# atsuki-ichikawa/KoeMorph

Measured on AMD Instinct MI355X. Metric: blendshape frames/sec (52-coef, 256-win, d_model=256), higher is better.
Workload: dtype f32; 1 GPU; C2: 256 windows/GPU x 136448 samples (8.5 s @16 kHz) -> 1024-pt STFT, hop 533, 80-bin log-mel (257 frames) -> dual-stream attention d_model=256, 8 heads, window 256 -> 52 coefficients + EMA; from audio resident in HBM (rotating batches); windows_per_gpu=256, samples_per_window=136448, parallelism=window-sharded x1, no collective

## Files before the change

koemorph_amd/csrc/km_api.hip:

```cpp
#include <hip/hip_runtime.h>

#include <cstdlib>

#include <cstring>
#include <vector>

#include "km_context.h"
#include "km_device.h"
#include "km_gemm.h"

using namespace km;

#define HIP_TRY(expr)                                                                         \
    do {                                                                                      \
        hipError_t e_ = (expr);                                                               \
        if (e_ != hipSuccess) {                                                                                                        \
            (void)hipGetLastError();  \
            return fail(KM_ERR_HIP, "%s: %s", #expr, hipGetErrorString(e_));                                                           \
        }                                                                                                                              \
    } while (0)

static int free_streams(Context* c);
static int free_train(Context* c);
static int free_pipeline(Context* c);
// ... 7 lines not shown
    return KM_OK;
}

static int need_dual(Context* c) {
    if (int rc = need_ready(c)) return rc;
    if (c->kind != 0) return fail(KM_ERR_INVALID_ARG, "this entry point needs a dual-stream handle (km_create), not a legacy one");
    return KM_OK;
}

static int need_legacy_train(Context* c, int64_t B) {
    if (int rc = need_ready(c)) return rc;
    if (c->kind != 1) return fail(KM_ERR_INVALID_ARG, "this entry point needs a legacy handle (km_legacy_create)");
    if (!c->tr_params || !c->ltr_ws) return fail(KM_ERR_NOT_FINALIZED, "call km_legacy_train_init first");
    if (B <= 0 || B > c->tr_windows) return fail(KM_ERR_WORKSPACE, "km_legacy_train_init sized the step for %lld windows, got %lld",
                                                 (long long)c->tr_windows, (long long)B);
    return KM_OK;
}

namespace km { LogParams plan_log_params(MelPlan* p); }

extern "C" {

int km_finalize(km_handle h, void* stream) {
    if (!h) return fail(KM_ERR_INVALID_ARG, "NULL handle");
    Context* c = h;
    int ndev = 0;
    if (hipGetDeviceCount(&ndev) != hipSuccess || ndev == 0)
        return fail(KM_ERR_HIP, "no HIP device: libkoemorph_hip has no CPU fallback");
    HIP_TRY(hipGetDevice(&c->device));
    if (!c->host_finalized)
        if (int rc = finalize_host(c)) return rc;
    for (auto& kv : c->packed) {
        Packed& p = kv.second;
        if (!p.dev) HIP_TRY(hipMalloc(reinterpret_cast<void**>(&p.dev), p.host.size() * sizeof(float)));
        HIP_TRY(hipMemcpyAsync(p.dev, p.host.data(), p.host.size() * sizeof(float), hipMemcpyHostToDevice,
                               (hipStream_t)stream));
    }
    HIP_TRY(hipStreamSynchronize((hipStream_t)stream));
    for (MelPlan* p : c->mel_plans)
        if (int rc = upload_mel_plan(p)) return rc;
    if (c->kind != 2)
        if (int rc = ensure_chunk_counters(c, 4096, stream)) return rc;
    c->dev_finalized = true;
    return KM_OK;
}

static int free_ws(Context* c) {
    if (c->ws_zemo) HIP_TRY(hipFree(c->ws_zemo));
    if (c->ws_zemo_win) HIP_TRY(hipFree(c->ws_zemo_win));
    if (c->ws_melpow) HIP_TRY(hipFree(c->ws_melpow));
    if (c->ws_melmax) HIP_TRY(hipFree(c->ws_melmax));
    if (c->ws_mel) HIP_TRY(hipFree(c->ws_mel));
    if (c->ws_short) HIP_TRY(hipFree(c->ws_short));
    if (c->ws_generic) HIP_TRY(hipFree(c->ws_generic));
    c->ws_zemo = c->ws_zemo_win = c->ws_melpow = c->ws_mel = c->ws_short = c->ws_generic = nullptr;
    c->ws_melmax = nullptr;
    c->ws_windows = c->ws_samples = c->ws_frames = 0;
    c->ws_mels = 0;
    return KM_OK;
}

int km_reserve(km_handle h, int64_t max_windows, int64_t max_samples) {
    if (!h || max_windows <= 0 || max_samples < 0) return fail(KM_ERR_INVALID_ARG, "km_reserve: bad argument");
    Context* c = h;
    if (c->kind == 2) return fail(KM_ERR_INVALID_ARG, "KoeMorphModel handles take no audio: use km_koemorph_reserve");
    int min_hop = c->cfg.mel.hop_length, max_mels = c->cfg.mel.n_mels;
// ... 1124 lines not shown
```

koemorph_amd/csrc/km_context.h:

```cpp
#pragma once

#include <cstdint>
#include <map>
#include <string>
#include <vector>

#include "koemorph.h"

namespace km {

constexpr int kNumMouth = 28;
constexpr int kNumExpr = 24;
extern const int kMouthIdx[kNumMouth];
extern const int kExprIdx[kNumExpr];

struct HostParam {
    std::vector<int64_t> shape;
    std::vector<float> data;
    bool loaded = false;
};

struct Packed {
    std::vector<float> host;
    float* dev = nullptr;
};

constexpr int kMelRpWaves = 8;
constexpr int kMelRpGroups = 4;
constexpr int kMelRpRow = 580;

struct MelPlan {
    km_mel_config cfg{};
    int n_freq = 0;
    std::vector<float> window;
    std::vector<float> twiddle;
    std::vector<int32_t> fb_start;
    std::vector<int32_t> fb_count;
    std::vector<int32_t> fb_offset;
    std::vector<float> fb_weight;
    std::vector<int32_t> fbg_gid;
    std::vector<int32_t> fbg_desc;
    std::vector<float> fbg_weight;
    int fbg_extent = 0;
    float* d_window = nullptr;
    float* d_twiddle = nullptr;
    int32_t* d_fb_start = nullptr;
    int32_t* d_fb_count = nullptr;
    int32_t* d_fb_offset = nullptr;
    float* d_fb_weight = nullptr;
    int32_t* d_fbg_gid = nullptr;
    int32_t* d_fbg_desc = nullptr;
    float* d_fbg_weight = nullptr;
    bool uploaded = false;
};

struct Options {
    int core_split = 0;
// ... 270 lines not shown
```

koemorph_amd/csrc/km_core.hip:

```cpp
#include <hip/hip_runtime.h>

#include <type_traits>

#include "km_context.h"
#include "km_device.h"

namespace km {

typedef float f32x4 __attribute__((ext_vector_type(4)));
#define KM_MFMA(a, b, c) __builtin_amdgcn_mfma_f32_16x16x4f32((a), (b), (c), 0, 0, 0)

#define HIP_TRY(expr)                                                                         \
    do {                                                                                      \
        hipError_t e_ = (expr);                                                               \
        if (e_ != hipSuccess) {                                                                                                        \
            (void)hipGetLastError();  \
            return fail(KM_ERR_HIP, "%s: %s", #expr, hipGetErrorString(e_));                                                           \
        }                                                                                                                              \
    } while (0)

namespace fused {
constexpr int D = 256, T = 256, NK = 80, NQ = 28, DH = 128;
constexpr int KT = 259, KTP = 264, YS = 264, NW = 8, NT = 512;
constexpr int KP = 33;
// ... 37 lines not shown
    const float* seq_edge;
    int seq_nfc, seq_stride, seq_n;
    const unsigned char* ready;
    unsigned char* started;
    const int* seq_start;
    int seq_min;
};

__device__ __forceinline__ int mouth_slot_of(int i) { return (i >= 14 && i <= 40) ? i - 14 : (i == 51 ? 27 : -1); }

template <bool ATTN, bool FUSE_DB, int NP = 0, bool TAB = false>
__global__ __launch_bounds__(512) void core_fused_kernel(CoreArgs a) {
    using namespace fused;
    extern __shared__ __attribute__((aligned(16))) float smem[];
    float* R1 = smem;
    float* R2 = smem + r1_floats(NP);

    const int b = blockIdx.x;
    const int tid = threadIdx.x;
    const int lane = tid & 63;
    const int wave = __builtin_amdgcn_readfirstlane(tid >> 6);
    const int g = lane >> 4, j = lane & 15;
    if constexpr (FUSE_DB) {
        if (a.ready && !a.ready[b]) return;
    }

    const int n0 = 32 * wave + j;
    float4 bw0 = make_float4(0.f, 0.f, 0.f, 0.f), bw1 = bw0;
    if constexpr (NP == 0) {
        const float4* wp0 = reinterpret_cast<const float4*>(a.wce_p) + (size_t)wave * KP * 64 + lane;
        bw0 = wp0[0];
    }
    const float bb0 = a.bce[n0], bb1 = a.bce[n0 + 16];
    const float g0 = a.ln_g[n0], g1 = a.ln_g[n0 + 16], be0 = a.ln_b[n0], be1 = a.ln_b[n0 + 16];
    float bf4[4], w24[4];
#pragma unroll
    for (int r = 0; r < 4; ++r) { bf4[r] = a.bf[16 * wave + 4 * g + r]; w24[r] = a.w2[16 * wave + 4 * g + r]; }
    const float tail_b2 = a.b2[0], tail_ws = tid < 52 ? a.wsum[tid] : 0.f;

    if constexpr (FUSE_DB) {
        float ref_db, floor_db;
        log_window_consts(a.lp, __uint_as_float(a.melmax[b]), ref_db, floor_db);
        const int F = a.n_frames;
        const int U = a.n_use;
        const int tv = U < T ? U : T;
        const float4* src = reinterpret_cast<const float4*>(a.melpow + (int64_t)b * F * NK);
        const float4 *seq_rows = nullptr, *seq_e = nullptr;
        if constexpr (TAB) {
            int r0 = a.seq_start[b];
            r0 = (r0 < 0 ? 0 : r0) - a.seq_min;
            r0 = r0 < 0 ? 0 : (r0 > a.seq_nfc - F ? a.seq_nfc - F : r0);
            seq_rows = reinterpret_cast<const float4*>(a.seq_pow + (int64_t)r0 * NK);
            seq_e = reinterpret_cast<const float4*>(a.seq_edge + (int64_t)b * 2 * NK);
        } else if (a.seq_pow) {
            const int64_t gw = a.win0 + b, clip = gw / a.seq_n, wi = gw - clip * a.seq_n;
            seq_rows = reinterpret_cast<const float4*>(a.seq_pow + (clip * a.seq_nfc + wi * a.seq_stride) * NK);
            seq_e = reinterpret_cast<const float4*>(a.seq_edge + gw * 2 * NK);
        }
        auto row4 = [&](int fr) -> const float4* {
            if (!seq_rows) return src + fr * 20;
            return fr == 0 ? seq_e : (fr == F - 1 ? seq_e + 20 : seq_rows + fr * 20);
        };
        float4* dst = reinterpret_cast<float4*>(R1);
        const float4 z4 = make_float4(0.f, 0.f, 0.f, 0.f);
        if constexpr (NP > 0) {
            auto src_row = [&](int t) -> int {
                if (t < T) return t < tv ? (t < F ? t : F - 1) : -1;
                if (t >= T + 3) return -1;
                const int r = t - T;
                int fr = -1;
                if (U >= 3) fr = U - 3 + r; else if (r < U) fr = r;
// ... 133 lines not shown
    } else {
        const float4* wp = reinterpret_cast<const float4*>(a.wce_p) + (size_t)wave * KP * 64 + lane;
        float4 bw = bw0;
        for (int kp = 0; kp < KP; ++kp) {
            const float4 bn = wp[(size_t)(kp + 1 < KP ? kp + 1 : kp) * 64];
#pragma unroll
            for (int ds = 0; ds < 2; ++ds) {
                const float* xr = R1 + (4 * (2 * kp + ds) + g) * NK + j;
                const float b0 = ds ? bw.z : bw.x, b1 = ds ? bw.w : bw.y;
                float av[5];
#pragma unroll
                for (int mt = 0; mt < 5; ++mt) av[mt] = xr[16 * mt];
#pragma unroll
                for (int mt = 0; mt < 5; ++mt) {
                    acc[mt][0] = KM_MFMA(av[mt], b0, acc[mt][0]);
                    acc[mt][1] = KM_MFMA(av[mt], b1, acc[mt][1]);
                }
            }
            bw = bn;
        }
    }
    f32x4 q0 = f32x4{0, 0, 0, 0}, q1 = q0, v0 = q0, v1 = q0;
    if constexpr (NP == 0) {
        const f32x4* qp0 = reinterpret_cast<const f32x4*>(a.qk_p) + (size_t)wave * KB * 2 * 64 + lane;
        const f32x4* vp0 = reinterpret_cast<const f32x4*>(a.wv_p) + (size_t)wave * KB * 2 * 64 + lane;
        q0 = qp0[0]; q1 = qp0[64]; v0 = vp0[0]; v1 = vp0[64];
    }
    {
#pragma unroll
        for (int mt = 0; mt < 5; ++mt)
#pragma unroll
            for (int r = 0; r < 4; ++r) { acc[mt][0][r] += bb0; acc[mt][1][r] += bb1; }
    }
    float mean[5][4], rstd[5][4];
#pragma unroll
    for (int pass = 0; pass < 2; ++pass) {
        float part[5][4];
#pragma unroll
        for (int mt = 0; mt < 5; ++mt)
#pragma unroll
            for (int r = 0; r < 4; ++r) {
                float v;
                if (pass == 0) {
                    v = acc[mt][0][r] + acc[mt][1][r];
                } else {
                    const float d0 = acc[mt][0][r] - mean[mt][r], d1 = acc[mt][1][r] - mean[mt][r];
                    v = d0 * d0 + d1 * d1;
                }
                part[mt][r] = row16_sum(v);
            }
        float* P = R2 + pass * (NW * NK);
        if (j == 0) {
#pragma unroll
            for (int mt = 0; mt < 5; ++mt)
#pragma unroll
                for (int r = 0; r < 4; ++r) P[(16 * mt + 4 * g + r) * NW + wave] = part[mt][r];
        }
        __syncthreads();
        float* Tt = R2 + 2 * NW * NK + pass * NK;
        if (lane < NK / NW) {
            const int row = wave * (NK / NW) + lane;
            const f32x4* pr = reinterpret_cast<const f32x4*>(P + row * NW);
            const f32x4 lo = pr[0], hi = pr[1];
            float s = 0.f;
            s += lo[0]; s += lo[1]; s += lo[2]; s += lo[3];
            s += hi[0]; s += hi[1]; s += hi[2]; s += hi[3];
            Tt[row] = s;
        }
        __syncthreads();
#pragma unroll
        for (int mt = 0; mt < 5; ++mt) {
            const f32x4 t4 = *reinterpret_cast<const f32x4*>(Tt + 16 * mt + 4 * g);
#pragma unroll
            for (int r = 0; r < 4; ++r) {
                if (pass == 0) mean[mt][r] = t4[r] * (1.0f / D);
                else rstd[mt][r] = __builtin_amdgcn_rsqf(t4[r] * (1.0f / D) + 1e-5f);
            }
        }
    }
    {
#pragma unroll
        for (int mt = 0; mt < 5; ++mt)
#pragma unroll
            for (int r = 0; r < 4; ++r) {
                const float y0 = (acc[mt][0][r] - mean[mt][r]) * rstd[mt][r] * g0 + be0;
                const float y1 = (acc[mt][1][r] - mean[mt][r]) * rstd[mt][r] * g1 + be1;
                if constexpr (NP == 0) {
                    float* yr = R1 + (16 * mt + 4 * g + r) * YS + n0;
                    yr[0] = y0;
                    yr[16] = y1;
                } else {
                    unsigned short* yp = reinterpret_cast<unsigned short*>(R1) + (16 * mt + 4 * g + r) * YSB + n0;
                    float r0 = y0, r1 = y1;
#pragma unroll
                    for (int pc = 0; pc < NP; ++pc) {
                        const __bf16 p0 = (__bf16)r0, p1 = (__bf16)r1;
                        yp[pc * (NK * YSB)] = __builtin_bit_cast(unsigned short, p0);
                        yp[pc * (NK * YSB) + 16] = __builtin_bit_cast(unsigned short, p1);
                        r0 -= (float)p0;
                        r1 -= (float)p1;
                    }
                }
            }
    }
    __syncthreads();

    f32x4 S[5][2], V[5][2];
#pragma unroll
    for (int mt = 0; mt < 5; ++mt) {
        S[mt][0] = f32x4{0, 0, 0, 0}; S[mt][1] = f32x4{0, 0, 0, 0};
        V[mt][0] = f32x4{0, 0, 0, 0}; V[mt][1] = f32x4{0, 0, 0, 0};
    }
    if constexpr (NP > 0) {
        const u32x4c* wp = reinterpret_cast<const u32x4c*>(a.qkv_s) + (size_t)wave * 8 * 4 * NP * 64 + lane;
        const unsigned short* Yp = reinterpret_cast<const unsigned short*>(R1) + j * YSB + 8 * g;
        u32x4c bw[4][NP];
#pragma unroll
        for (int t = 0; t < 4; ++t)
#pragma unroll
            for (int pc = 0; pc < NP; ++pc) bw[t][pc] = wp[(t * NP + pc) * 64];
        for (int kb = 0; kb < 8; ++kb) {
            const int kn = kb + 1 < 8 ? kb + 1 : kb;
            u32x4c bn[4][NP];
#pragma unroll
            for (int t = 0; t < 4; ++t)
#pragma unroll
                for (int pc = 0; pc < NP; ++pc) bn[t][pc] = wp[((kn * 4 + t) * NP + pc) * 64];
#pragma unroll
            for (int mt = 0; mt < 5; ++mt) {
                bf16x8 ap[NP];
#pragma unroll
                for (int pc = 0; pc < NP; ++pc)
                    ap[pc] = __builtin_bit_cast(bf16x8, *reinterpret_cast<const u32x4c*>(Yp + pc * (NK * YSB) + 16 * mt * YSB + 32 * kb));
#pragma unroll
                for (int t = 0; t < 4; ++t) {
                    f32x4 c4 = t < 2 ? S[mt][t] : V[mt][t - 2];
                    if constexpr (NP == 3) {
                        c4 = __builtin_amdgcn_mfma_f32_16x16x32_bf16(ap[1], __builtin_bit_cast(bf16x8, bw[t][1]), c4, 0, 0, 0);
                        c4 = __builtin_amdgcn_mfma_f32_16x16x32_bf16(ap[0], __builtin_bit_cast(bf16x8, bw[t][2]), c4, 0, 0, 0);
                        c4 = __builtin_amdgcn_mfma_f32_16x16x32_bf16(ap[2], __builtin_bit_cast(bf16x8, bw[t][0]), c4, 0, 0, 0);
                    }
                    c4 = __builtin_amdgcn_mfma_f32_16x16x32_bf16(ap[0], __builtin_bit_cast(bf16x8, bw[t][1]), c4, 0, 0, 0);
                    c4 = __builtin_amdgcn_mfma_f32_16x16x32_bf16(ap[1], __builtin_bit_cast(bf16x8, bw[t][0]), c4, 0, 0, 0);
                    c4 = __builtin_amdgcn_mfma_f32_16x16x32_bf16(ap[0], __builtin_bit_cast(bf16x8, bw[t][0]), c4, 0, 0, 0);
                    if (t < 2) S[mt][t] = c4; else V[mt][t - 2] = c4;
                }
            }
#pragma unroll
            for (int t = 0; t < 4; ++t)
#pragma unroll
                for (int pc = 0; pc < NP; ++pc) bw[t][pc] = bn[t][pc];
        }
    } else {
        const f32x4* qp = reinterpret_cast<const f32x4*>(a.qk_p) + (size_t)wave * KB * 2 * 64 + lane;
        const f32x4* vp = reinterpret_cast<const f32x4*>(a.wv_p) + (size_t)wave * KB * 2 * 64 + lane;
        for (int kb = 0; kb < KB; ++kb) {
            const int kn = kb + 1 < KB ? kb + 1 : kb;
            const f32x4 q0n = qp[(size_t)kn * 128], q1n = qp[(size_t)kn * 128 + 64];
            const f32x4 v0n = vp[(size_t)kn * 128], v1n = vp[(size_t)kn * 128 + 64];
            f32x4 ya[5];
#pragma unroll
            for (int mt = 0; mt < 5; ++mt)
                ya[mt] = *reinterpret_cast<const f32x4*>(R1 + (16 * mt + j) * YS + 16 * kb + 4 * g);
#pragma unroll
            for (int s = 0; s < 4; ++s)
#pragma unroll
                for (int mt = 0; mt < 5; ++mt) {
                    const float av = ya[mt][s];
                    S[mt][0] = KM_MFMA(av, q0[s], S[mt][0]);
                    S[mt][1] = KM_MFMA(av, q1[s], S[mt][1]);
                    V[mt][0] = KM_MFMA(av, v0[s], V[mt][0]);
                    V[mt][1] = KM_MFMA(av, v1[s], V[mt][1]);
                }
            q0 = q0n; q1 = q1n; v0 = v0n; v1 = v1n;
        }
    }
#pragma unroll
    for (int qt = 0; qt < 2; ++qt) {
        float m = S[0][qt][0];
#pragma unroll
        for (int mt = 0; mt < 5; ++mt)
#pragma unroll
            for (int r = 0; r < 4; ++r) m = fmaxf(m, S[mt][qt][r]);
        m = fmaxf(m, __shfl_xor(m, 16));
        m = fmaxf(m, __shfl_xor(m, 32));
        float sum = 0.f;
#pragma unroll
        for (int mt = 0; mt < 5; ++mt)
#pragma unroll
            for (int r = 0; r < 4; ++r) {
                const float e = __builtin_amdgcn_exp2f((S[mt][qt][r] - m) * 1.44269504088896341f);
                S[mt][qt][r] = e;
                sum += e;
            }
        sum += __shfl_xor(sum, 16);
        sum += __shfl_xor(sum, 32);
        const float inv = __builtin_amdgcn_rcpf(sum);
#pragma unroll
        for (int mt = 0; mt < 5; ++mt)
#pragma unroll
            for (int r = 0; r < 4; ++r) S[mt][qt][r] *= inv;
    }

    f32x4 O[2][2];
    O[0][0] = f32x4{0, 0, 0, 0}; O[0][1] = f32x4{0, 0, 0, 0};
    O[1][0] = f32x4{0, 0, 0, 0}; O[1][1] = f32x4{0, 0, 0, 0};
#pragma unroll
// ... 43 lines not shown
    Z[0] = f32x4{0, 0, 0, 0}; Z[1] = f32x4{0, 0, 0, 0};
    {
        const f32x4* fp = reinterpret_cast<const f32x4*>(a.wf_p) + (size_t)wave * KB * 64 + lane;
#pragma unroll 4
        for (int kb = 0; kb < KB; ++kb) {
            const f32x4 wa = fp[(size_t)kb * 64];
            const f32x4 o0 = *reinterpret_cast<const f32x4*>(R1 + j * YS + 16 * kb + 4 * g);
            const f32x4 o1 = *reinterpret_cast<const f32x4*>(R1 + (16 + j) * YS + 16 * kb + 4 * g);
#pragma unroll
            for (int s = 0; s < 4; ++s) {
                Z[0] = KM_MFMA(wa[s], o0[s], Z[0]);
                Z[1] = KM_MFMA(wa[s], o1[s], Z[1]);
            }
        }
    }
    {
        float zp[2] = {0.f, 0.f};
#pragma unroll
        for (int r = 0; r < 4; ++r) {
            const float bfv = bf4[r], w2v = w24[r];
            zp[0] += fmaxf(Z[0][r] + bfv, 0.f) * w2v;
            zp[1] += fmaxf(Z[1][r] + bfv, 0.f) * w2v;
        }
#pragma unroll
        for (int qt = 0; qt < 2; ++qt) {
            zp[qt] += __shfl_xor(zp[qt], 16);
            zp[qt] += __shfl_xor(zp[qt], 32);
        }
        if (g == 0) { R2[wave * 32 + j] = zp[0]; R2[wave * 32 + 16 + j] = zp[1]; }
    }
    __syncthreads();
    if (tid < 52) {
        const int slot = mouth_slot_of(tid);
        float z;
        if (slot >= 0) {
            z = tail_b2;
#pragma unroll
            for (int w = 0; w < NW; ++w) z += R2[w * 32 + slot];
        } else {
            z = a.zemo[(a.win0 + b) / a.zemo_div];
        }
        const float bs = 1.0f / (1.0f + expf(-z));
        float val = fminf(fmaxf(tail_ws * bs, 0.f), 1.f);
        if (a.raw) a.raw[(int64_t)b * 52 + tid] = bs;
        if (a.state) {
            float* st = a.state + (int64_t)b * 52 + tid;
            const bool first = a.started ? !a.started[b] : (a.first != 0);
            if (!first) val = a.alpha * val + (1.0f - a.alpha) * (*st);
            *st = val;
        }
        a.out[(int64_t)b * 52 + tid] = val;
    }
    if constexpr (FUSE_DB) {
        __syncthreads();
        if (tid == 0 && a.started) a.started[b] = 1;
    }
}

constexpr int EWPB = 4;
constexpr int ENT = 1024;
constexpr int EKQ1 = 4;
constexpr int EKQ2 = 8;

__global__ __launch_bounds__(1024) void emotion_kernel(const float* __restrict__ emo, int64_t B, int ED, int d, int DH,
                                                       const float* __restrict__ wee_t, const float* __restrict__ bee,
                                                       const float* __restrict__ lg, const float* __restrict__ lb,
                                                       const float* __restrict__ we2, const float* __restrict__ be2,
                                                       const float* __restrict__ w2, const float* __restrict__ b2,
                                                       float* __restrict__ zemo) {
    extern __shared__ __attribute__((aligned(16))) float es[];
    float* emo_s = es;
    float* e1 = emo_s + EWPB * ED;
    float* part = e1 + EWPB * d;
    const int tid = threadIdx.x, lane = tid & 63, wave = tid >> 6;
    const int64_t b0 = (int64_t)blockIdx.x * EWPB;
    const int nb = (int)((B - b0) < EWPB ? (B - b0) : EWPB);
    for (int i = tid; i < EWPB * ED; i += ENT) {
        const int w = i / ED;
        emo_s[i] = w < nb ? emo[b0 * ED + i] : 0.f;
    }
    __syncthreads();
    {
        const int kq = tid >> 8, kchunk = (ED + EKQ1 - 1) / EKQ1;
        const int k0 = kq * kchunk, k1 = (k0 + kchunk) < ED ? (k0 + kchunk) : ED;
        for (int n = tid & 255; n < d; n += 256) {
            float acc[EWPB];
#pragma unroll
// ... 212 lines not shown
    if (lds > 160 * 1024) return fail(KM_ERR_UNSUPPORTED, "emotion_dim/d_model too large for the emotion kernel");
    static PerDeviceOnce once;
    if (once.first(c->device))
        HIP_TRY(hipFuncSetAttribute(reinterpret_cast<const void*>(&emotion_kernel),
                                    hipFuncAttributeMaxDynamicSharedMemorySize, 160 * 1024));
    const unsigned grid = (unsigned)((B + EWPB - 1) / EWPB);
    if (c->d == 256 && c->DH == 128 && c->ED <= 256) {
        hipLaunchKernelGGL(emotion_kernel_d256, dim3(grid), dim3(ENT), 0, (hipStream_t)stream, emo, B, c->ED,
                           dv(c, "wee_t"), dv(c, "bee"), dv(c, "eln_g"), dv(c, "eln_b"), dv(c, "we2"), dv(c, "be2"),
                           dv(c, "w2"), dv(c, "b2"), zemo);
        HIP_TRY(hipGetLastError());
        return KM_OK;
    }
    hipLaunchKernelGGL(emotion_kernel, dim3(grid), dim3(ENT), lds, (hipStream_t)stream, emo, B, c->ED, c->d, c->DH,
                       dv(c, "wee_t"), dv(c, "bee"), dv(c, "eln_g"), dv(c, "eln_b"), dv(c, "we2"), dv(c, "be2"),
                       dv(c, "w2"), dv(c, "b2"), zemo);
    HIP_TRY(hipGetLastError());
    return KM_OK;
}

static int core_attrs(Context* c) {
    static PerDeviceOnce once;
    if (once.first(c->device)) {
        const struct { const void* fn; int lds; } kernels[] = {
            {(const void*)&core_fused_kernel<false, false>, fused::LDS_BYTES}, {(const void*)&core_fused_kernel<true, false>, fused::LDS_BYTES},
            {(const void*)&core_fused_kernel<false, true>, fused::LDS_BYTES}, {(const void*)&core_fused_kernel<false, true, 2>, fused::lds_bytes(2)},
            {(const void*)&core_fused_kernel<false, true, 3>, fused::lds_bytes(3)}, {(const void*)&core_fused_kernel<false, true, 0, true>, fused::LDS_BYTES}};
        for (const auto& k : kernels) HIP_TRY(hipFuncSetAttribute(k.fn, hipFuncAttributeMaxDynamicSharedMemorySize, k.lds));
    }
    return KM_OK;
}

static void core_weights(Context* c, CoreArgs& a) {
    a.wce_p = dv(c, "wce_p"); a.bce = dv(c, "bce"); a.ln_g = dv(c, "ln_g"); a.ln_b = dv(c, "ln_b");
    a.qk_p = dv(c, "qk_p"); a.wv_p = dv(c, "wv_p"); a.wf_p = dv(c, "wf_p"); a.bf = dv(c, "bf");
    a.w2 = dv(c, "w2"); a.b2 = dv(c, "b2"); a.wsum = dv(c, "wsum");
    a.alpha = c->alpha;
}

int launch_core_fused(Context* c, const float* mel, int64_t B, int64_t T_in, const float* mel_short,
                      const float* zemo, float* out, float* raw, float* attn, float* state, int first,
                      void* stream) {
    if (int rc = core_attrs(c)) return rc;
    CoreArgs a{};
    core_weights(c, a);
    a.mel = mel; a.mel_short = mel_short; a.zemo = zemo; a.t_in = (int)T_in;
    a.out = out; a.raw = raw; a.attn = attn; a.state = state; a.first = first; a.win0 = 0; a.zemo_div = 1;
    if (attn)
        hipLaunchKernelGGL((core_fused_kernel<true, false>), dim3((unsigned)B), dim3(fused::NT), fused::LDS_BYTES, (hipStream_t)stream, a);
    else
        hipLaunchKernelGGL((core_fused_kernel<false, false>), dim3((unsigned)B), dim3(fused::NT), fused::LDS_BYTES, (hipStream_t)stream, a);
    HIP_TRY(hipGetLastError());
    return KM_OK;
}

LogParams plan_log_params(MelPlan* p);

__global__ __launch_bounds__(64) void seq_window_max_kernel(const unsigned* __restrict__ fmax, const unsigned* __restrict__ emax,
                                                            unsigned* __restrict__ melmax, int64_t win0, int nfc, int stride,
                                                            int n_per_clip, int n_frames) {
    const int64_t gw = win0 + blockIdx.x, clip = gw / n_per_clip, wi = gw - clip * n_per_clip;
    const unsigned* f = fmax + clip * nfc + wi * stride;
    unsigned m = 0;
    for (int r = 1 + threadIdx.x; r < n_frames - 1; r += 64) m = max(m, f[r]);
    if (threadIdx.x < 2) m = max(m, emax[gw * 2 + threadIdx.x]);
#pragma unroll
    for (int o = 32; o > 0; o >>= 1) m = max(m, (unsigned)__shfl_xor((int)m, o));
    if (threadIdx.x == 0) melmax[blockIdx.x] = m;
// ... 36 lines not shown
    }
}

int launch_clip_window_max(Context* c, const float* span, const float* edge, const int* start, int64_t B, int min_start,
                           int64_t n_span, int n_frames, void* stream) {
    if (!span || !edge || !start || B <= 0 || n_frames < 3 || n_span < n_frames || c->NK % 4 != 0)
        return fail(KM_ERR_INVALID_ARG, "clip window maximum: bad argument");
    hipLaunchKernelGGL(clip_window_max_kernel, dim3((unsigned)B), dim3(CWM_NT), 0, (hipStream_t)stream, span, edge, start, c->ws_melmax,
                       min_start, (int)n_span, n_frames, c->NK / 4);
    HIP_TRY(hipGetLastError());
    return KM_OK;
}

int launch_core_fused_db(Context* c, MelPlan* p, int64_t B, int64_t n_frames, const float* zemo, float* out, void* stream,
                         const CoreSrc& src) {
    if (int rc = core_attrs(c)) return rc;
    CoreArgs a{};
    core_weights(c, a);
    a.zemo = zemo; a.t_in = (int)n_frames;
    a.out = out; a.state = src.state; a.first = src.first; a.win0 = src.win0; a.zemo_div = src.zemo_div > 0 ? src.zemo_div : 1;
    a.melpow = c->ws_melpow; a.melmax = c->ws_melmax; a.n_frames = (int)n_frames; a.lp = plan_log_params(p);
    a.n_use = (int)(src.n_use > 0 ? src.n_use : n_frames); a.ready = src.ready; a.started = src.started;
    if (const SeqCore* s = src.seq) { a.seq_pow = s->pow; a.seq_edge = s->edge; a.seq_nfc = s->nfc; a.seq_stride = s->stride; a.seq_n = s->n_per_clip; }
    if (const ClipTable* t = src.tab) {
        if (src.seq || c->opt.core_split == 3 || c->opt.core_split == 6)
            return fail(KM_ERR_UNSUPPORTED, "fused core: a start-frame table goes with neither strided images nor the split-bf16 variant");
        a.seq_pow = t->span; a.seq_edge = t->edge; a.seq_nfc = t->n_span; a.seq_stride = 0; a.seq_n = 1;
        a.seq_start = t->start; a.seq_min = t->min_start;
        hipLaunchKernelGGL((core_fused_kernel<false, true, 0, true>), dim3((unsigned)B), dim3(fused::NT), fused::LDS_BYTES, (hipStream_t)stream, a);
        HIP_TRY(hipGetLastError());
        return KM_OK;
    }
    const int terms = c->opt.core_split;
    if (terms == 3) {
        a.qkv_s = dv(c, "qkv_s2"); a.wce_s = dv(c, "wce_s2");
        hipLaunchKernelGGL((core_fused_kernel<false, true, 2>), dim3((unsigned)B), dim3(fused::NT), fused::lds_bytes(2), (hipStream_t)stream, a);
    } else if (terms == 6) {
        a.qkv_s = dv(c, "qkv_s3"); a.wce_s = dv(c, "wce_s3");
        hipLaunchKernelGGL((core_fused_kernel<false, true, 3>), dim3((unsigned)B), dim3(fused::NT), fused::lds_bytes(3), (hipStream_t)stream, a);
    } else {
        hipLaunchKernelGGL((core_fused_kernel<false, true>), dim3((unsigned)B), dim3(fused::NT), fused::LDS_BYTES, (hipStream_t)stream, a);
    }
    HIP_TRY(hipGetLastError());
    return KM_OK;
}

__global__ void ema_scan_kernel(float* __restrict__ x, int64_t B, int64_t N, int nb, float alpha) {
    const int64_t i = (int64_t)blockIdx.x * blockDim.x + threadIdx.x;
    if (i >= B * nb) return;
    const int64_t b = i / nb;
    const int cidx = (int)(i - b * nb);
    float* p = x + b * N * nb + cidx;
    float prev = p[0];
    for (int64_t t = 1; t < N; ++t) {
        const float v = alpha * p[t * nb] + (1.0f - alpha) * prev;
        p[t * nb] = v;
        prev = v;
    }
}

int launch_ema_scan(Context* c, float* x, int64_t B, int64_t N, void* stream) {
    const int64_t n = B * c->NB;
    hipLaunchKernelGGL(ema_scan_kernel, dim3((unsigned)((n + 127) / 128)), dim3(128), 0, (hipStream_t)stream, x, B, N,
                       c->NB, c->alpha);
    HIP_TRY(hipGetLastError());
    return KM_OK;
// ... 12 lines not shown
```

koemorph_amd/csrc/km_host.cpp:

```cpp
#include <cctype>
#include <cmath>
#include <cstdlib>
#include <cstdarg>
#include <cstdio>
#include <cstring>

#include "km_context.h"
#include "km_kmmf.h"

namespace km {

const int kMouthIdx[kNumMouth] = {14, 15, 16, 17, 18, 19, 20, 21, 22, 23, 24, 25, 26, 27,
                                  28, 29, 30, 31, 32, 33, 34, 35, 36, 37, 38, 39, 40, 51};
const int kExprIdx[kNumExpr] = {0, 1, 2, 3, 4, 5, 6, 7, 8, 9, 10, 11, 12, 13,
                                41, 42, 43, 44, 45, 46, 47, 48, 49, 50};

static thread_local char g_err[512] = "";

void set_error(const char* fmt, ...) {
    va_list ap;
    va_start(ap, fmt);
    vsnprintf(g_err, sizeof(g_err), fmt, ap);
    va_end(ap);
}
// ... 19 lines not shown
            const double a = A[(size_t)i * K + k];
            const double* b = &B[(size_t)k * N];
            double* c = &C[(size_t)i * N];
            for (int j = 0; j < N; ++j) c[j] += a * b[j];
        }
    return C;
}

static inline uint16_t bf16_rne(float f) {
    uint32_t u;
    std::memcpy(&u, &f, 4);
    return (uint16_t)((u + 0x7FFFu + ((u >> 16) & 1u)) >> 16);
}
static inline float bf16_to_float(uint16_t h) {
    const uint32_t u = (uint32_t)h << 16;
    float f;
    std::memcpy(&f, &u, 4);
    return f;
}

static dvec transpose(const dvec& A, int R, int Cn) {
    dvec T((size_t)R * Cn);
    for (int i = 0; i < R; ++i)
        for (int j = 0; j < Cn; ++j) T[(size_t)j * R + i] = A[(size_t)i * Cn + j];
    return T;
}

static std::vector<float> to_f(const dvec& v) { return std::vector<float>(v.begin(), v.end()); }

static const std::vector<float>& P(Context* c, const char* k) { return c->params.at(k).data; }

static void put(Context* c, const char* name, std::vector<float>&& v) {
    c->packed[name].host = std::move(v);
}

static dvec softmax_d(const std::vector<float>& w, double temp) {
    dvec r(w.size());
    double m = -1e300;
    for (float x : w) m = std::fmax(m, x / temp);
    double s = 0;
    for (size_t i = 0; i < w.size(); ++i) { r[i] = std::exp(w[i] / temp - m); s += r[i]; }
    for (double& x : r) x /= s;
    return r;
}

static void fold_chain(const dvec& bin, const dvec& Wa, const dvec& ba, const dvec& Wb, const dvec& bb,
                       const dvec& W1, const dvec& b1, int d, int DH, dvec& F, dvec& f) {
    dvec WaT = transpose(Wa, d, d), WbT = transpose(Wb, d, d), W1T = transpose(W1, DH, d);
    dvec M2 = mm(WaT, WbT, d, d, d);
    F = mm(M2, W1T, d, d, DH);
    dvec t1 = mm(bin, WaT, 1, d, d);
    for (int i = 0; i < d; ++i) t1[i] += ba[i];
    dvec t2 = mm(t1, WbT, 1, d, d);
    for (int i = 0; i < d; ++i) t2[i] += bb[i];
    f = mm(t2, W1T, 1, d, DH);
    for (int i = 0; i < DH; ++i) f[i] += b1[i];
}

static void pack_frag(const std::vector<float>& W, int N, int K, int Kpad, float* dst);

int finalize_host_legacy(Context* c) {
    const int d = c->d, hd = c->hd, NQ = c->NB;
    const dvec inw = to_d(P(c, "attention.in_proj_weight")), inb = to_d(P(c, "attention.in_proj_bias"));
    dvec Wq(inw.begin(), inw.begin() + (size_t)d * d);
    dvec Q = mm(to_d(P(c, "blendshape_queries")), transpose(Wq, d, d), NQ, d, d);
    const double scale = 1.0 / std::sqrt((double)hd);
// ... 259 lines not shown
    put(c, "be2", to_f(bfE));
    put(c, "wee_t", to_f(transpose(to_d(P(c, "emotion_encoder.weight")), d, ED)));
    if (d == 256 && ED <= 256) {
        std::vector<float> wpad((size_t)256 * d, 0.0f);
        const std::vector<float>& wt = c->packed.at("wee_t").host;
        std::copy(wt.begin(), wt.end(), wpad.begin());
        put(c, "wee_t256", std::move(wpad));
    }
    put(c, "bee", std::vector<float>(P(c, "emotion_encoder.bias")));
    put(c, "eln_g", std::vector<float>(P(c, "emotion_norm.weight")));
    put(c, "eln_b", std::vector<float>(P(c, "emotion_norm.bias")));
    put(c, "bce", std::vector<float>(P(c, "mel_channel_encoder.bias")));
    put(c, "ln_g", std::vector<float>(P(c, "mel_norm.weight")));
    put(c, "ln_b", std::vector<float>(P(c, "mel_norm.bias")));
    put(c, "w2", std::vector<float>(P(c, "blendshape_decoder.3.weight")));
    put(c, "b2", std::vector<float>(P(c, "blendshape_decoder.3.bias")));
    put(c, "wsum", std::move(wsum));
    put(c, "wce_raw", std::vector<float>(P(c, "mel_channel_encoder.weight")));
    put(c, "wv_raw", to_f(Wv));

    c->fused_ok = (d == 256 && H == 8 && c->T == 256 && c->NK == 80 && NB == 52 && c->cfg.mel_temporal_frames == 3);
    if (c->fused_ok) {
        const std::vector<float>& Wce = P(c, "mel_channel_encoder.weight");
        const int NW = 8, KP = 33;
        std::vector<float> wce_p((size_t)NW * KP * 64 * 4);
        for (int w = 0; w < NW; ++w)
            for (int kp = 0; kp < KP; ++kp)
                for (int l = 0; l < 64; ++l)
                    for (int e = 0; e < 4; ++e) {
                        const int g = l >> 4, j = l & 15, ds = e >> 1, t = e & 1;
                        const int k = 4 * (2 * kp + ds) + g, n = 16 * (2 * w + t) + j;
                        wce_p[(((size_t)w * KP + kp) * 64 + l) * 4 + e] = k < KT ? Wce[(size_t)n * KT + k] : 0.0f;
                    }
        put(c, "wce_p", std::move(wce_p));

        const int KB = d / 16;
        std::vector<float> qk_p((size_t)H * KB * 2 * 64 * 4), wv_p((size_t)H * KB * 2 * 64 * 4), wf_p((size_t)8 * KB * 64 * 4);
        for (int h = 0; h < H; ++h)
            for (int kb = 0; kb < KB; ++kb)
                for (int t = 0; t < 2; ++t)
                    for (int l = 0; l < 64; ++l)
                        for (int s = 0; s < 4; ++s) {
                            const int g = l >> 4, j = l & 15, k = 16 * kb + 4 * g + s;
                            const size_t o = ((((size_t)h * KB + kb) * 2 + t) * 64 + l) * 4 + s;
                            const int q = 16 * t + j;
                            qk_p[o] = q < NQ ? (float)Qk[((size_t)h * NQ + q) * d + k] : 0.0f;
                            wv_p[o] = (float)Wv[(size_t)(h * hd + 16 * t + j) * d + k];
                        }
        for (int w = 0; w < 8; ++w)
            for (int kb = 0; kb < KB; ++kb)
                for (int l = 0; l < 64; ++l)
                    for (int s = 0; s < 4; ++s) {
                        const int g = l >> 4, j = l & 15, k = 16 * kb + 4 * g + s;
                        wf_p[(((size_t)w * KB + kb) * 64 + l) * 4 + s] = (float)Wf[(size_t)k * DH + 16 * w + j];
                    }
        put(c, "qk_p", std::move(qk_p));
        put(c, "wv_p", std::move(wv_p));
        put(c, "wf_p", std::move(wf_p));
        for (int NP = 2; NP <= 3; ++NP) {
            std::vector<uint16_t> img((size_t)H * 8 * 4 * NP * 64 * 8);
            for (int h = 0; h < H; ++h)
                for (int kb = 0; kb < 8; ++kb)
                    for (int t = 0; t < 4; ++t)
                        for (int l = 0; l < 64; ++l)
                            for (int e = 0; e < 8; ++e) {
                                const int g = l >> 4, j = l & 15, k = 32 * kb + 8 * g + e, q = 16 * (t & 1) + j;
                                float w = t < 2 ? (q < NQ ? (float)Qk[((size_t)h * NQ + q) * d + k] : 0.0f)
                                                : (float)Wv[(size_t)(h * hd + 16 * (t & 1) + j) * d + k];
                                for (int pc = 0; pc < NP; ++pc) {
                                    const uint16_t b16 = bf16_rne(w);
                                    img[(((((size_t)h * 8 + kb) * 4 + t) * NP + pc) * 64 + l) * 8 + e] = b16;
                                    w -= bf16_to_float(b16);
                                }
                            }
            std::vector<float> bits(img.size() / 2);
            std::memcpy(bits.data(), img.data(), img.size() * sizeof(uint16_t));
            put(c, NP == 2 ? "qkv_s2" : "qkv_s3", std::move(bits));
            std::vector<uint16_t> enc((size_t)8 * 9 * 2 * NP * 64 * 8);
            for (int w = 0; w < 8; ++w)
                for (int kb = 0; kb < 9; ++kb)
                    for (int t = 0; t < 2; ++t)
                        for (int l = 0; l < 64; ++l)
                            for (int e = 0; e < 8; ++e) {
                                const int g = l >> 4, j = l & 15, k = 32 * kb + 8 * g + e, n = 32 * w + 16 * t + j;
                                float wv = k < KT ? Wce[(size_t)n * KT + k] : 0.0f;
                                for (int pc = 0; pc < NP; ++pc) {
                                    const uint16_t b16 = bf16_rne(wv);
                                    enc[(((((size_t)w * 9 + kb) * 2 + t) * NP + pc) * 64 + l) * 8 + e] = b16;
                                    wv -= bf16_to_float(b16);
                                }
                            }
// ... 434 lines not shown
```

Before: 1.812 million frames/s.

## Fold LayerNorm mean and affine into precomputed weights for fp32 fused core

For the fp32 (NP==0) fused path, the channel-encoder weights and bias are column-mean-centered on the host so the LayerNorm mean is zero by construction. The gain is folded into the Q/V projection weights and the beta term into the output bias. The kernel now computes only a sum-of-squares reduction, defers the per-row rstd scaling to after the Q/V MFMAs, and drops one reduction pass and its barriers. Tail loads (zemo, EMA state) are hoisted to kernel start and a final syncthreads is removed, at the cost of different float rounding from the precomputed centering.

```diff
diff --git a/koemorph_amd/csrc/km_api.hip b/koemorph_amd/csrc/km_api.hip
--- a/koemorph_amd/csrc/km_api.hip
+++ b/koemorph_amd/csrc/km_api.hip
@@ -63,6 +63,7 @@
         if (int rc = finalize_host(c)) return rc;
     for (auto& kv : c->packed) {
         Packed& p = kv.second;
+        if (p.host_only) continue;
         if (!p.dev) HIP_TRY(hipMalloc(reinterpret_cast<void**>(&p.dev), p.host.size() * sizeof(float)));
         HIP_TRY(hipMemcpyAsync(p.dev, p.host.data(), p.host.size() * sizeof(float), hipMemcpyHostToDevice,
                                (hipStream_t)stream));
diff --git a/koemorph_amd/csrc/km_context.h b/koemorph_amd/csrc/km_context.h
--- a/koemorph_amd/csrc/km_context.h
+++ b/koemorph_amd/csrc/km_context.h
@@ -23,6 +23,7 @@
 struct Packed {
     std::vector<float> host;
     float* dev = nullptr;
+    bool host_only = false;
 };
 
 constexpr int kMelRpWaves = 8;
diff --git a/koemorph_amd/csrc/km_core.hip b/koemorph_amd/csrc/km_core.hip
--- a/koemorph_amd/csrc/km_core.hip
+++ b/koemorph_amd/csrc/km_core.hip
@@ -93,11 +93,21 @@
         bw0 = wp0[0];
     }
     const float bb0 = a.bce[n0], bb1 = a.bce[n0 + 16];
-    const float g0 = a.ln_g[n0], g1 = a.ln_g[n0 + 16], be0 = a.ln_b[n0], be1 = a.ln_b[n0 + 16];
+    float g0 = 1.f, g1 = 1.f, be0 = 0.f, be1 = 0.f;
+    if constexpr (NP > 0) { g0 = a.ln_g[n0]; g1 = a.ln_g[n0 + 16]; be0 = a.ln_b[n0]; be1 = a.ln_b[n0 + 16]; }
     float bf4[4], w24[4];
 #pragma unroll
     for (int r = 0; r < 4; ++r) { bf4[r] = a.bf[16 * wave + 4 * g + r]; w24[r] = a.w2[16 * wave + 4 * g + r]; }
     const float tail_b2 = a.b2[0], tail_ws = tid < 52 ? a.wsum[tid] : 0.f;
+    float tail_z = 0.f, tail_st = 0.f;
+    bool tail_first = a.first != 0;
+    if (tid < 52) {
+        if (mouth_slot_of(tid) < 0) tail_z = a.zemo[(a.win0 + b) / a.zemo_div];
+        if (a.state) {
+            tail_st = a.state[(int64_t)b * 52 + tid];
+            if (a.started) tail_first = !a.started[b];
+        }
+    }
 
     if constexpr (FUSE_DB) {
         float ref_db, floor_db;
@@ -297,64 +307,81 @@
 #pragma unroll
             for (int r = 0; r < 4; ++r) { acc[mt][0][r] += bb0; acc[mt][1][r] += bb1; }
     }
-    float mean[5][4], rstd[5][4];
-#pragma unroll
-    for (int pass = 0; pass < 2; ++pass) {
+    if constexpr (NP == 0) {
         float part[5][4];
 #pragma unroll
         for (int mt = 0; mt < 5; ++mt)
 #pragma unroll
+            for (int r = 0; r < 4; ++r) part[mt][r] = row16_sum(acc[mt][0][r] * acc[mt][0][r] + acc[mt][1][r] * acc[mt][1][r]);
+        if (j == 0) {
+#pragma unroll
+            for (int mt = 0; mt < 5; ++mt)
+#pragma unroll
+                for (int r = 0; r < 4; ++r) R2[(16 * mt + 4 * g + r) * NW + wave] = part[mt][r];
+        }
+        __syncthreads();
+#pragma unroll
+        for (int mt = 0; mt < 5; ++mt)
+#pragma unroll
             for (int r = 0; r < 4; ++r) {
-                float v;
-                if (pass == 0) {
-                    v = acc[mt][0][r] + acc[mt][1][r];
-                } else {
-                    const float d0 = acc[mt][0][r] - mean[mt][r], d1 = acc[mt][1][r] - mean[mt][r];
-                    v = d0 * d0 + d1 * d1;
+                float* yr = R1 + (16 * mt + 4 * g + r) * YS + n0;
+                yr[0] = acc[mt][0][r];
+                yr[16] = acc[mt][1][r];
+            }
+    } else {
+        float mean[5][4], rstd[5][4];
+#pragma unroll
+        for (int pass = 0; pass < 2; ++pass) {
+            float part[5][4];
+#pragma unroll
+            for (int mt = 0; mt < 5; ++mt)
+#pragma unroll
+                for (int r = 0; r < 4; ++r) {
+                    float v;
+                    if (pass == 0) {
+                        v = acc[mt][0][r] + acc[mt][1][r];
+                    } else {
+                        const float d0 = acc[mt][0][r] - mean[mt][r], d1 = acc[mt][1][r] - mean[mt][r];
+                        v = d0 * d0 + d1 * d1;
+                    }
+                    part[mt][r] = row16_sum(v);
                 }
-                part[mt][r] = row16_sum(v);
-            }
-        float* P = R2 + pass * (NW * NK);
-        if (j == 0) {
+            float* P = R2 + pass * (NW * NK);
+            if (j == 0) {
+#pragma unroll
+                for (int mt = 0; mt < 5; ++mt)
+#pragma unroll
+                    for (int r = 0; r < 4; ++r) P[(16 * mt + 4 * g + r) * NW + wave] = part[mt][r];
+            }
+            __syncthreads();
+            float* Tt = R2 + 2 * NW * NK + pass * NK;
+            if (lane < NK / NW) {
+                const int row = wave * (NK / NW) + lane;
+                const f32x4* pr = reinterpret_cast<const f32x4*>(P + row * NW);
+                const f32x4 lo = pr[0], hi = pr[1];
+                float s = 0.f;
+                s += lo[0]; s += lo[1]; s += lo[2]; s += lo[3];
+                s += hi[0]; s += hi[1]; s += hi[2]; s += hi[3];
+                Tt[row] = s;
+            }
+            __syncthreads();
+#pragma unroll
+            for (int mt = 0; mt < 5; ++mt) {
+                const f32x4 t4 = *reinterpret_cast<const f32x4*>(Tt + 16 * mt + 4 * g);
+#pragma unroll
+                for (int r = 0; r < 4; ++r) {
+                    if (pass == 0) mean[mt][r] = t4[r] * (1.0f / D);
+                    else rstd[mt][r] = __builtin_amdgcn_rsqf(t4[r] * (1.0f / D) + 1e-5f);
+                }
+            }
+        }
+        {
 #pragma unroll
             for (int mt = 0; mt < 5; ++mt)
 #pragma unroll
-                for (int r = 0; r < 4; ++r) P[(16 * mt + 4 * g + r) * NW + wave] = part[mt][r];
-        }
-        __syncthreads();
-        float* Tt = R2 + 2 * NW * NK + pass * NK;
-        if (lane < NK / NW) {
-            const int row = wave * (NK / NW) + lane;
-            const f32x4* pr = reinterpret_cast<const f32x4*>(P + row * NW);
-            const f32x4 lo = pr[0], hi = pr[1];
-            float s = 0.f;
-            s += lo[0]; s += lo[1]; s += lo[2]; s += lo[3];
-            s += hi[0]; s += hi[1]; s += hi[2]; s += hi[3];
-            Tt[row] = s;
-        }
-        __syncthreads();
-#pragma unroll
-        for (int mt = 0; mt < 5; ++mt) {
-            const f32x4 t4 = *reinterpret_cast<const f32x4*>(Tt + 16 * mt + 4 * g);
-#pragma unroll
-            for (int r = 0; r < 4; ++r) {
-                if (pass == 0) mean[mt][r] = t4[r] * (1.0f / D);
-                else rstd[mt][r] = __builtin_amdgcn_rsqf(t4[r] * (1.0f / D) + 1e-5f);
-            }
-        }
-    }
-    {
-#pragma unroll
-        for (int mt = 0; mt < 5; ++mt)
-#pragma unroll
-            for (int r = 0; r < 4; ++r) {
-                const float y0 = (acc[mt][0][r] - mean[mt][r]) * rstd[mt][r] * g0 + be0;
-                const float y1 = (acc[mt][1][r] - mean[mt][r]) * rstd[mt][r] * g1 + be1;
-                if constexpr (NP == 0) {
-                    float* yr = R1 + (16 * mt + 4 * g + r) * YS + n0;
-                    yr[0] = y0;
-                    yr[16] = y1;
-                } else {
+                for (int r = 0; r < 4; ++r) {
+                    const float y0 = (acc[mt][0][r] - mean[mt][r]) * rstd[mt][r] * g0 + be0;
+                    const float y1 = (acc[mt][1][r] - mean[mt][r]) * rstd[mt][r] * g1 + be1;
                     unsigned short* yp = reinterpret_cast<unsigned short*>(R1) + (16 * mt + 4 * g + r) * YSB + n0;
                     float r0 = y0, r1 = y1;
 #pragma unroll
@@ -366,7 +393,7 @@
                         r1 -= (float)p1;
                     }
                 }
-            }
+        }
     }
     __syncthreads();
 
@@ -417,6 +444,21 @@
                 for (int pc = 0; pc < NP; ++pc) bw[t][pc] = bn[t][pc];
         }
     } else {
+        {
+            float* Tw = R2 + NW * NK + wave * NK;
+#pragma unroll
+            for (int u = 0; u < 2; ++u) {
+                const int row = 64 * u + lane;
+                if (row < NK) {
+                    const f32x4* pr = reinterpret_cast<const f32x4*>(R2 + row * NW);
+                    const f32x4 lo = pr[0], hi = pr[1];
+                    float s = 0.f;
+                    s += lo[0]; s += lo[1]; s += lo[2]; s += lo[3];
+                    s += hi[0]; s += hi[1]; s += hi[2]; s += hi[3];
+                    Tw[row] = s;
+                }
+            }
+        }
         const f32x4* qp = reinterpret_cast<const f32x4*>(a.qk_p) + (size_t)wave * KB * 2 * 64 + lane;
         const f32x4* vp = reinterpret_cast<const f32x4*>(a.wv_p) + (size_t)wave * KB * 2 * 64 + lane;
         for (int kb = 0; kb < KB; ++kb) {
@@ -438,6 +480,18 @@
                     V[mt][1] = KM_MFMA(av, v1[s], V[mt][1]);
                 }
             q0 = q0n; q1 = q1n; v0 = v0n; v1 = v1n;
+        }
+        __builtin_amdgcn_wave_barrier();
+        const float* Tw = R2 + NW * NK + wave * NK;
+#pragma unroll
+        for (int mt = 0; mt < 5; ++mt) {
+            const f32x4 t4 = *reinterpret_cast<const f32x4*>(Tw + 16 * mt + 4 * g);
+#pragma unroll
+            for (int r = 0; r < 4; ++r) {
+                const float rs = __builtin_amdgcn_rsqf(t4[r] * (1.0f / D) + 1e-5f);
+                S[mt][0][r] *= rs; S[mt][1][r] *= rs;
+                V[mt][0][r] *= rs; V[mt][1][r] *= rs;
+            }
         }
     }
 #pragma unroll
@@ -547,27 +601,22 @@
     __syncthreads();
     if (tid < 52) {
         const int slot = mouth_slot_of(tid);
-        float z;
+        float z = tail_z;
         if (slot >= 0) {
             z = tail_b2;
 #pragma unroll
             for (int w = 0; w < NW; ++w) z += R2[w * 32 + slot];
-        } else {
-            z = a.zemo[(a.win0 + b) / a.zemo_div];
         }
         const float bs = 1.0f / (1.0f + expf(-z));
         float val = fminf(fmaxf(tail_ws * bs, 0.f), 1.f);
         if (a.raw) a.raw[(int64_t)b * 52 + tid] = bs;
         if (a.state) {
-            float* st = a.state + (int64_t)b * 52 + tid;
-            const bool first = a.started ? !a.started[b] : (a.first != 0);
-            if (!first) val = a.alpha * val + (1.0f - a.alpha) * (*st);
-            *st = val;
+            if (!tail_first) val = a.alpha * val + (1.0f - a.alpha) * tail_st;
+            a.state[(int64_t)b * 52 + tid] = val;
         }
         a.out[(int64_t)b * 52 + tid] = val;
     }
     if constexpr (FUSE_DB) {
-        __syncthreads();
         if (tid == 0 && a.started) a.started[b] = 1;
     }
 }
@@ -846,8 +895,8 @@
 }
 
 static void core_weights(Context* c, CoreArgs& a) {
-    a.wce_p = dv(c, "wce_p"); a.bce = dv(c, "bce"); a.ln_g = dv(c, "ln_g"); a.ln_b = dv(c, "ln_b");
-    a.qk_p = dv(c, "qk_p"); a.wv_p = dv(c, "wv_p"); a.wf_p = dv(c, "wf_p"); a.bf = dv(c, "bf");
+    a.wce_p = dv(c, "wce_cp"); a.bce = dv(c, "bce_c");
+    a.qk_p = dv(c, "qk_gp"); a.wv_p = dv(c, "wv_gp"); a.wf_p = dv(c, "wf_p"); a.bf = dv(c, "bf_ln");
     a.w2 = dv(c, "w2"); a.b2 = dv(c, "b2"); a.wsum = dv(c, "wsum");
     a.alpha = c->alpha;
 }
@@ -950,6 +999,10 @@
         return KM_OK;
     }
     const int terms = c->opt.core_split;
+    if (terms == 3 || terms == 6) {
+        a.wce_p = a.qk_p = a.wv_p = nullptr;
+        a.bce = dv(c, "bce"); a.ln_g = dv(c, "ln_g"); a.ln_b = dv(c, "ln_b"); a.bf = dv(c, "bf");
+    }
     if (terms == 3) {
         a.qkv_s = dv(c, "qkv_s2"); a.wce_s = dv(c, "wce_s2");
         hipLaunchKernelGGL((core_fused_kernel<false, true, 2>), dim3((unsigned)B), dim3(fused::NT), fused::lds_bytes(2), (hipStream_t)stream, a);
diff --git a/koemorph_amd/csrc/km_host.cpp b/koemorph_amd/csrc/km_host.cpp
--- a/koemorph_amd/csrc/km_host.cpp
+++ b/koemorph_amd/csrc/km_host.cpp
@@ -75,6 +75,11 @@
 
 static void put(Context* c, const char* name, std::vector<float>&& v) {
     c->packed[name].host = std::move(v);
+}
+
+static void put_host(Context* c, const char* name, std::vector<float>&& v) {
+    put(c, name, std::move(v));
+    c->packed[name].host_only = true;
 }
 
 static dvec softmax_d(const std::vector<float>& w, double temp) {
@@ -400,7 +405,34 @@
                         const int k = 4 * (2 * kp + ds) + g, n = 16 * (2 * w + t) + j;
                         wce_p[(((size_t)w * KP + kp) * 64 + l) * 4 + e] = k < KT ? Wce[(size_t)n * KT + k] : 0.0f;
                     }
-        put(c, "wce_p", std::move(wce_p));
+        put_host(c, "wce_p", std::move(wce_p));
+
+        const dvec lg = to_d(P(c, "mel_norm.weight")), lb = to_d(P(c, "mel_norm.bias"));
+        {
+            dvec colmean(KT, 0.0);
+            for (int k = 0; k < KT; ++k) {
+                double s = 0;
+                for (int n = 0; n < d; ++n) s += (double)Wce[(size_t)n * KT + k];
+                colmean[k] = s / d;
+            }
+            std::vector<float> wce_cp((size_t)NW * KP * 64 * 4);
+            for (int w = 0; w < NW; ++w)
+                for (int kp = 0; kp < KP; ++kp)
+                    for (int l = 0; l < 64; ++l)
+                        for (int e = 0; e < 4; ++e) {
+                            const int g = l >> 4, j = l & 15, ds = e >> 1, t = e & 1;
+                            const int k = 4 * (2 * kp + ds) + g, n = 16 * (2 * w + t) + j;
+                            wce_cp[(((size_t)w * KP + kp) * 64 + l) * 4 + e] = k < KT ? (float)((double)Wce[(size_t)n * KT + k] - colmean[k]) : 0.0f;
+                        }
+            put(c, "wce_cp", std::move(wce_cp));
+            const std::vector<float>& bce = P(c, "mel_channel_encoder.bias");
+            double bm = 0;
+            for (int n = 0; n < d; ++n) bm += (double)bce[n];
+            bm /= d;
+            std::vector<float> bce_c(d);
+            for (int n = 0; n < d; ++n) bce_c[n] = (float)((double)bce[n] - bm);
+            put(c, "bce_c", std::move(bce_c));
+        }
 
         const int KB = d / 16;
         std::vector<float> qk_p((size_t)H * KB * 2 * 64 * 4), wv_p((size_t)H * KB * 2 * 64 * 4), wf_p((size_t)8 * KB * 64 * 4);
@@ -422,9 +454,32 @@
                         const int g = l >> 4, j = l & 15, k = 16 * kb + 4 * g + s;
                         wf_p[(((size_t)w * KB + kb) * 64 + l) * 4 + s] = (float)Wf[(size_t)k * DH + 16 * w + j];
                     }
-        put(c, "qk_p", std::move(qk_p));
-        put(c, "wv_p", std::move(wv_p));
+        put_host(c, "qk_p", std::move(qk_p));
+        put_host(c, "wv_p", std::move(wv_p));
         put(c, "wf_p", std::move(wf_p));
+        {
+            std::vector<float> qk_gp((size_t)H * KB * 2 * 64 * 4), wv_gp((size_t)H * KB * 2 * 64 * 4);
+            for (int h = 0; h < H; ++h)
+                for (int kb = 0; kb < KB; ++kb)
+                    for (int t = 0; t < 2; ++t)
+                        for (int l = 0; l < 64; ++l)
+                            for (int s = 0; s < 4; ++s) {
+                                const int g = l >> 4, j = l & 15, k = 16 * kb + 4 * g + s;
+                                const size_t o = ((((size_t)h * KB + kb) * 2 + t) * 64 + l) * 4 + s;
+                                const int q = 16 * t + j;
+                                qk_gp[o] = q < NQ ? (float)(lg[k] * Qk[((size_t)h * NQ + q) * d + k]) : 0.0f;
+                                wv_gp[o] = (float)(lg[k] * Wv[(size_t)(h * hd + 16 * t + j) * d + k]);
+                            }
+            put(c, "qk_gp", std::move(qk_gp));
+            put(c, "wv_gp", std::move(wv_gp));
+            dvec bf_ln = bf;
+            for (int i = 0; i < d; ++i) {
+                double cv = 0;
+                for (int k = 0; k < d; ++k) cv += lb[k] * Wv[(size_t)i * d + k];
+                for (int u = 0; u < DH; ++u) bf_ln[u] += cv * Wf[(size_t)i * DH + u];
+            }
+            put(c, "bf_ln", to_f(bf_ln));
+        }
         for (int NP = 2; NP <= 3; ++NP) {
             std::vector<uint16_t> img((size_t)H * 8 * 4 * NP * 64 * 8);
             for (int h = 0; h < H; ++h)
```

After: 1.830 million frames/s (median of 3 runs). Within noise of the previous version (+1.0%).
